# yefeng22222/RUB_MIMO

Measured on AMD Instinct MI355X. Metric: complex IQ samples/s through 4x4 MMSE detect; EVM-dB delta vs CPU ref, higher is better.
Workload: dtype fp32 (complex64; fp64 weight solve)

## Files before the change

rub_mimo_amd/csrc/engine.cpp:

```cpp
#include <mutex>

#include "engine_internal.hpp"

namespace {

thread_local std::string g_err;

std::mutex g_tw_mu;
float2 *g_tw = nullptr;
int g_tw_dev = -1;

}

namespace mimo {

int host_fail(int code, const char *msg) {
  g_err = msg;
  return code;
}

int get_twiddles(float2 **out) {
  std::lock_guard<std::mutex> lk(g_tw_mu);
  int dev = 0;
  HIPCHK(hipGetDevice(&dev));
// ... 163 lines not shown
  h->siso_tx = cfg->siso_tx; h->siso_rx = cfg->siso_rx;
  h->thr = cfg->plateau_threshold;
  h->cfo = cfg->cfo_correct != 0;
  h->qam = make_qam(q);
  h->acb = (uint64_t)h->SL * (h->nac * N + 4);
  h->txl = (uint64_t)h->pid * h->SL;
  h->win_len = h->acb + h->txl;
  h->dn = 1.0f / sqrtf((float)h->M_occ);
  h->ls_scale = h->dn / (float)h->nac;
  h->nv_norm = (h->nac >= 2) ? ((double)h->dn * (double)h->dn /
                                ((double)h->M_occ * N * N * (h->nac - 1)))
                             : 0.0;
  uint32_t F = 1;
  while (F < 2 * h->SL + h->M - 1 || F < 2 * h->M) F <<= 1;
  h->search_ls = F <= 16384 && search_ls_supported(ilog2(F), ilog2(h->M));
  if (!h->search_ls) {
    F = 1;
    while (F < h->SL + h->M - 1) F <<= 1;
    if (F > 8192) F = 8192;
    if (F < 2 * h->M) F = 2 * h->M;
  }
  h->F = F; h->log2F = ilog2(F);
  h->lagc = F - h->M + 1;
  h->n_lagc = (h->SL + h->lagc - 1) / h->lagc;
  h->n_slots = N * h->nac + 1;
  if (hip_stream) {
    h->stream = (hipStream_t)hip_stream;
  } else {
    if (hipStreamCreateWithFlags(&h->stream, hipStreamNonBlocking) != hipSuccess) {
      delete h;
      return fail(MIMO_ERR_HIP, "hipStreamCreate failed");
    }
    h->own_stream = true;
  }
  {
    int dev = 0, ncu = 0;
    if (hipGetDevice(&dev) == hipSuccess &&
        hipDeviceGetAttribute(&ncu, hipDeviceAttributeMultiprocessorCount, dev) == hipSuccess &&
        ncu > 0)
      h->n_cu = (uint32_t)ncu;
  }
  rc = get_twiddles(&h->tw);
  if (!rc) rc = build_codes(h->codes, h->M, N, h->nac, h->p.data(), cfg->s0_bits, cfg->s1_bits,
                            h->log2F, true, h->stream);
  if (rc) { mimo_rx_destroy(h); return rc; }
  uint32_t m_s0 = 0;
  for (uint32_t i = 0; i < h->M; i += 2) if (h->p[i] != MIMO_SC_NULL) m_s0++;
  std::vector<float> vs(h->n_slots);
  const double FF = (double)F * (double)F, MM = (double)h->M * (double)h->M;
  vs[0] = (float)((double)m_s0 / (MM * FF));
  for (uint32_t sl = 1; sl < h->n_slots; sl++) vs[sl] = (float)(1.0 / ((double)h->M * FF));
  if (ls_window_supported(h->log2M, h->nac, false)) {
    const uint32_t T = h->M / 8;
    std::vector<int8_t> sw(sign.size());
    for (size_t row = 0; row < (size_t)N * h->nac; row++)
      for (uint32_t lt = 0; lt < T; lt++)
        for (uint32_t e = 0; e < 8; e++) sw[row * h->M + 8 * lt + e] = sign[row * h->M + lt + T * e];
    if (h->s1sign_w.ensure(sw.size()) != hipSuccess ||
        hipMemcpy(h->s1sign_w.p, sw.data(), sw.size(), hipMemcpyHostToDevice) != hipSuccess) {
      mimo_rx_destroy(h);
      return fail(MIMO_ERR_HIP, "table upload failed");
    }
  }
  if (h->vscale.ensure(h->n_slots) != hipSuccess || h->s1sign.ensure(sign.size()) != hipSuccess ||
      h->occ.ensure(h->M) != hipSuccess ||
      hipMemcpy(h->vscale.p, vs.data(), sizeof(float) * vs.size(), hipMemcpyHostToDevice) !=
          hipSuccess ||
      hipMemcpy(h->s1sign.p, sign.data(), sign.size(), hipMemcpyHostToDevice) != hipSuccess ||
      hipMemcpy(h->occ.p, h->occ_index.data(), sizeof(int32_t) * h->M, hipMemcpyHostToDevice) !=
          hipSuccess) {
    mimo_rx_destroy(h);
    return fail(MIMO_ERR_HIP, "table upload failed");
  }
  *out = h;
  return MIMO_OK;
}

int mimo_rx_destroy(mimo_rx *h) {
  if (!h) return MIMO_OK;
  if (h->stream) (void)hipStreamSynchronize(h->stream);
  close_debug_files(h);
  for (auto &e : h->timer.ev) {
    (void)hipEventDestroy(e.second.first);
    (void)hipEventDestroy(e.second.second);
  }
  for (auto &g : h->graphs)
    if (g.exec) (void)hipGraphExecDestroy(g.exec);
  if (h->own_stream && h->stream) (void)hipStreamDestroy(h->stream);
  delete h;
  return MIMO_OK;
}

int mimo_rx_set_callback(mimo_rx *h, mimo_rx_symbol_cb cb, void *user) {
  if (!h) return fail(MIMO_ERR_ARG, "null handle");
  h->cb = cb;
  h->user = user;
  return MIMO_OK;
}

int mimo_rx_set_siso(mimo_rx *h, uint32_t tx, uint32_t rx) {
  if (!h || tx >= h->N || rx >= h->N) return fail(MIMO_ERR_ARG, "siso index out of range");
  if (tx != h->siso_tx || rx != h->siso_rx) invalidate_graph(h);
  h->siso_tx = tx;
  h->siso_rx = rx;
  return MIMO_OK;
}

int mimo_rx_set_grid_cus(mimo_rx *h, uint32_t n_cu) {
  if (!h) return fail(MIMO_ERR_ARG, "null handle");
  int dev = 0, ncu = 0;
  if (n_cu == 0 && hipGetDevice(&dev) == hipSuccess &&
// ... 263 lines not shown
```

rub_mimo_amd/csrc/engine_diag.cpp:

```cpp
#include "engine_internal.hpp"

namespace mimo {

const DiagEnv &diag_env() {
  static const DiagEnv env = [] {
    auto on = [](const char *name) { const char *e = getenv(name); return e && e[0] == '1'; };
    DiagEnv d{};
    const char *e = getenv("RMIMO_SC_DIAG");
    d.sc_diag = e ? atoi(e) : 0;
    d.sc_prof = on("RMIMO_SC_PROF");
    d.sc_one_phase = on("RMIMO_SC_PHASES");
    d.sc_count = on("RMIMO_SC_COUNT");
    d.sc_count_items = d.sc_count && getenv("RMIMO_SC_COUNT")[1] == '+';
    e = getenv("RMIMO_LS_FORM");
    d.ls_terms = e && strcmp(e, "terms") == 0;
    d.dec_prof = on("RMIMO_DEC_PROF");
    d.cfo_debug = on("RMIMO_CFO_DEBUG");
    d.no_graph = on("RMIMO_NO_GRAPH") || d.sc_prof || d.dec_prof;
    return d;
  }();
  return env;
}

int diag_sc_prof_arm(mimo_rx *h, bool screen, hipStream_t s, unsigned long long **prof) {
  if (!diag_env().sc_prof) return MIMO_OK;
  if (!h->sc_prof.p) HIPCHK(h->sc_prof.ensure(32));
  HIPCHK(hipMemsetAsync(h->sc_prof.p, 0, 32 * sizeof(unsigned long long), s));
  HIPCHK(hipMemsetAsync(h->sc_prof.p + 8, 0xFF, sizeof(unsigned long long), s));
  if (screen) HIPCHK(hipMemsetAsync(h->sc_prof.p, 0xFF, sizeof(unsigned long long), s));
  *prof = h->sc_prof.p;
  return MIMO_OK;
}

int diag_sc_count(mimo_rx *h, uint32_t F, uint64_t nchunks, bool screen, uint32_t hot_cap,
                  hipStream_t s) {
  if (!diag_env().sc_count) return MIMO_OK;
  hipStreamCaptureStatus cst = hipStreamCaptureStatusNone;
  (void)hipStreamIsCapturing(s, &cst);
  if (cst != hipStreamCaptureStatusNone) return MIMO_OK;
  uint32_t q[2] = {0, 0};
  HIPCHK(hipMemcpyAsync(q, h->ws.queue.p, sizeof(q), hipMemcpyDeviceToHost, s));
  HIPCHK(hipStreamSynchronize(s));
  fprintf(stderr, "sc_count hot_items %u (screen %d, frames %u, chunks %llu)\n", q[1],
          screen ? 1 : 0, F, (unsigned long long)nchunks);
  if (!diag_env().sc_count_items || !screen) return MIMO_OK;
  const uint32_t n = std::min(q[1], hot_cap);
  std::vector<ScHot> hv(n);
  std::vector<unsigned long long> mn((size_t)F * nchunks), mx((size_t)F * nchunks);
  HIPCHK(hipMemcpyAsync(hv.data(), h->ws.hot.p, sizeof(ScHot) * n, hipMemcpyDeviceToHost, s));
  HIPCHK(hipMemcpyAsync(mn.data(), h->ws.scr_min.p, sizeof(unsigned long long) * mn.size(),
                        hipMemcpyDeviceToHost, s));
  HIPCHK(hipMemcpyAsync(mx.data(), h->ws.scr_max.p, sizeof(unsigned long long) * mx.size(),
                        hipMemcpyDeviceToHost, s));
  HIPCHK(hipStreamSynchronize(s));
  for (uint32_t i = 0; i < n; i++) {
    const ScHot &it = hv[i];
    const size_t ci = (size_t)it.f * nchunks + it.chunk;
    const long long lo = (long long)mn[ci] - it.w0, hi = (long long)mx[ci] - it.w0;
    const long long a0 = std::max<long long>(0, (lo - (long long)h->cp - 2) / kScIterLen);
    const long long a1 = std::min<long long>(kScSpan / kScIterLen - 1, hi / kScIterLen);
    fprintf(stderr, "sc_item %u f %u chunk %llu w0 %lld c0 %lld unproven [%lld, %lld] (%lld) "
            "iterations %lld-%lld\n", i, it.f, (unsigned long long)it.chunk, (long long)it.w0,
            (long long)it.c0, lo, hi, hi - lo + 1, a0, a1);
  }
  return MIMO_OK;
}

int diag_sc_prof_report(mimo_rx *h, bool screen, hipStream_t s) {
  if (!diag_env().sc_prof) return MIMO_OK;
  if (screen) {
    unsigned long long v[32];
// ... 8 lines not shown
            v[6], v[6] ? (double)v[10] / v[6] / 100.0 : 0.0,
            v[12] ? (double)v[11] / v[12] / 100.0 : 0.0, v[12], (double)(v[13] >> 32) / 100.0,
            (v[13] >> 24) & 0xFF, (double)(v[13] & 0xFFFFFF) / 100.0, v[14] >> 32,
            v[14] & 0xFFFFFFFFull, v[15]);
    const double np = v[4] ? (double)v[4] : 1.0;
    fprintf(stderr, "exact_split record %.2f us setup %.2f us iterations %.2f us (%.2f per pass) "
            "start offset avg %.2f max %.2f us | per iteration: ring %.2f scan %.2f walk %.2f us "
            "(first iteration's ring %.2f us per pass; guarded fills %llu)\n",
            v[20] / np / 100.0, v[21] / np / 100.0,
            v[22] / np / 100.0, v[23] / np, (v[26] / np - (double)v[0]) / 100.0,
            (double)(v[25] - v[0]) / 100.0, v[23] ? v[16] / (double)v[23] / 100.0 : 0.0,
            v[23] ? v[17] / (double)v[23] / 100.0 : 0.0, v[23] ? v[18] / (double)v[23] / 100.0 : 0.0,
            v[19] / np / 100.0, v[24]);
    fprintf(stderr, "exact_windows max per iteration %llu, iterations with >= 2 windows %llu "
            "(their passes' max duration %.2f us)\n", v[27], v[28], (double)v[29] / 100.0);
  } else {
    unsigned long long v[20];
    HIPCHK(hipMemcpyAsync(v, h->sc_prof.p, sizeof(v), hipMemcpyDeviceToHost, s));
    HIPCHK(hipStreamSynchronize(s));
    const double it = v[0] ? (double)v[0] : 1.0;
    fprintf(stderr, "sc_prof items %llu skipped %llu antenna_passes %llu cycles/item rows %.0f "
            "words %.0f resolve %.0f total %.0f wall_us/item %.2f span_us %.2f max_item_us %.2f "
            "last_start_us %.2f\n", v[0], v[6], v[1],
            v[2] / it, v[3] / it, v[4] / it, v[5] / it, v[7] / it / 100.0,
            (double)(v[9] - v[8]) / 100.0, v[10] / 100.0, (double)(v[11] - v[8]) / 100.0);
    fprintf(stderr, "sc_prof phases/item warm %.0f A %.0f scan %.0f B %.0f run %.0f | resolve "
            "passes %llu chain cycles/pass %.0f samples/pass %.1f\n",
            v[12] / it, v[13] / it, v[14] / it, v[15] / it, v[16] / it, v[17],
            v[17] ? (double)v[18] / v[17] : 0.0, v[17] ? (double)v[19] / v[17] : 0.0);
  }
  return MIMO_OK;
}

int diag_dec_prof_arm(mimo_rx *h, hipStream_t s, unsigned long long **prof) {
  if (!diag_env().dec_prof) return MIMO_OK;
  if (!h->sc_prof.p) HIPCHK(h->sc_prof.ensure(28));
  HIPCHK(hipMemsetAsync(h->sc_prof.p, 0, 8 * sizeof(unsigned long long), s));
  *prof = h->sc_prof.p;
  return MIMO_OK;
}

int diag_dec_prof_report(mimo_rx *h, hipStream_t s) {
  if (!diag_env().dec_prof) return MIMO_OK;
  unsigned long long v[8];
  HIPCHK(hipMemcpyAsync(v, h->sc_prof.p, sizeof(v), hipMemcpyDeviceToHost, s));
  HIPCHK(hipStreamSynchronize(s));
  const double it = v[0] ? (double)v[0] : 1.0;
  fprintf(stderr, "dec_prof items %llu cycles/item load %.0f fft %.0f apply %.0f reduce %.0f "
          "| stream split: pass0 %.0f fetch %.0f subfft %.0f\n",
          v[0], v[1] / it, v[2] / it, v[3] / it, v[4] / it, v[5] / it, v[6] / it, v[7] / it);
  return MIMO_OK;
}

int diag_cfo_frames(mimo_rx *h, uint32_t F, hipStream_t s) {
  if (!diag_env().cfo_debug || !h->cfo) return MIMO_OK;
  std::vector<FrameInfo> fi(F);
  HIPCHK(hipMemcpyAsync(fi.data(), h->ws.info.p, sizeof(FrameInfo) * F, hipMemcpyDeviceToHost, s));
  HIPCHK(hipStreamSynchronize(s));
  for (uint32_t f = 0; f < F; f++)
    fprintf(stderr, "cfo_dbg f %u status %d base %lld i0 %u eps %.9f E %lld\n", f, (int)fi[f].status,
            (long long)fi[f].base, fi[f].i0, (double)fi[f].cfo_eps, (long long)fi[f].cfo_E);
  return MIMO_OK;
}

}
```

rub_mimo_amd/csrc/engine_internal.hpp:

```cpp
#pragma once

#include <hip/hip_runtime.h>

#include <algorithm>
#include <array>
#include <cmath>
#include <cstdio>
#include <cstdlib>
#include <cstring>
#include <string>
#include <utility>
#include <vector>

#include "../../include/mimo_rx.h"
#include "kernels.hpp"

using namespace mimo;

#pragma GCC visibility push(hidden)
namespace mimo {

inline int fail(int code, const std::string &msg) { return host_fail(code, msg.c_str()); }

#define HIPCHK(x)                                                                       \
// ... 83 lines not shown
    return b.ensure(cnt);
  }
  uint32_t rec_frames = 0;
  uint64_t rec_stride = 0;
  DevBuf<unsigned long long> trig, keys;
  DevBuf<ScRecord> rec;
  DevBuf<FrameInfo> info;
  DevBuf<float2> G, W;
  DevBuf<float> gain;
  DevBuf<double> nvp, evm_part, evm_out, evm_chunk, lspart;
  DevBuf<uint32_t> evm_cnt;
  DevBuf<uint32_t> nrec;
  DevBuf<float2> lsq;
  DevBuf<unsigned long long> n_exact;
  DevBuf<uint32_t> queue;
  DevBuf<ScHot> hot;
  DevBuf<uint32_t> scr_flag;
  DevBuf<unsigned long long> scr_min, scr_max;
  DevBuf<unsigned long long> cand;
  DevBuf<unsigned long long> certfail;
  DevBuf<float2> spec;
  DevBuf<float2> wide;
  DevBuf<float2> cfo_iq;
  DevBuf<double> cfo_eps;
};

}
#pragma GCC visibility pop

struct mimo_rx {
  uint32_t M = 0, cp = 0, SL = 0, N = 0, nac = 0, pid = 0;
  uint32_t M_null = 0, M_pilot = 0, M_data = 0, M_occ = 0;
  int log2M = 0, log2F = 0;
  uint32_t F = 0, lagc = 0, n_lagc = 0, n_slots = 0;
  bool search_ls = false;
  bool cfo = false;
  uint32_t n_cu = 256;
  int det = 0;
  float noise_var = -1.0f;
  int keep_bias = 1;
  uint32_t siso_tx = 0, siso_rx = 0;
  double thr = 0.95;
  Qam qam{};
  uint64_t acb = 0, txl = 0, win_len = 0;
  float dn = 1.0f, ls_scale = 1.0f;
  double nv_norm = 0.0;
  std::vector<uint8_t> p;
  std::vector<int32_t> occ_index;
  hipStream_t stream = nullptr;
  bool own_stream = false;
  float2 *tw = nullptr;
  Codes codes;
  DevBuf<float> vscale;
  DevBuf<int8_t> s1sign, s1sign_w;
  DevBuf<int32_t> occ;
  Workspace ws;
  uint32_t last_frames = 0, last_max_out = 0;
  int last_decode_path = MIMO_DECODE_NONE;
  int last_cfo_mode = 0;
  uint32_t last_layout = 0;
  DevBuf<float> nu;
  DevBuf<float2> sic_T, sic_C;
  DevBuf<uint8_t> sic_order, sic_ok;
  DevBuf<float> sic_nu;
  DevBuf<float2> capbuf;
  uint64_t cap_len = 0, total = 0, origin = 0;
  uint64_t trim_clo = ~0ull;
  DevBuf<uint32_t> probe;
  int state = MIMO_STATE_SEEK_PLATEAU;
  uint64_t nsp = 0;
  bool have_sync = false, have_est = false;
  FrameInfo sinfo{};
  DevBuf<float2> symbuf;
  std::vector<float2> symhost;
  mimo_rx_symbol_cb cb = nullptr;
  void *user = nullptr;
  std::string dbg_dir;
  std::vector<FILE *> dbg_fsc;
  DevBuf<float> dbg_y, dbg_corr;
  DevBuf<unsigned long long> sc_prof;
  StageTimer timer;
  struct GraphEntry {
    mimo_batch key{};
    hipStream_t stream = nullptr;
    uint64_t gen = 0;
    hipGraphExec_t exec = nullptr;
    uint64_t used = 0;
  };
  std::array<GraphEntry, 4> graphs{};
  uint64_t graph_tick = 0;
};

struct mimo_tx {
  uint32_t M = 0, cp = 0, SL = 0, N = 0, nac = 0, M_occ = 0;
  int log2M = 0;
  float dn = 1.0f;
  hipStream_t stream = nullptr;
  Codes codes;
  std::vector<float2> s0, s1;
  DevBuf<int32_t> occ_list;
  DevBuf<float2> din, dout;
  float2 *tw = nullptr;
};

#pragma GCC visibility push(hidden)
namespace mimo {

int get_twiddles(float2 **out);
Qam make_qam(uint32_t order);
int validate_sctype(const uint8_t *p, uint32_t M, uint32_t *n0, uint32_t *n1, uint32_t *n2);
int build_codes(Codes &c, uint32_t M, uint32_t N, uint32_t nac, const uint8_t *p,
                const uint8_t *s0_bits, const uint8_t *s1_bits, int log2F, bool spectra,
                hipStream_t s);
int copy_W(mimo_rx *h, uint32_t f, float *W);
int copy_corr(mimo_rx *h, uint32_t F, uint32_t *corr, uint32_t *s0);

int ensure_workspace(mimo_rx *h, uint32_t F, uint64_t chunks);
double sc_band(uint32_t M);
struct SyncRequest {
  uint64_t chunk_lo;
  bool reset_trig;
  uint32_t fpc;
  const uint64_t *ref_starts;
  uint32_t ref_stride;
  bool zero_keys;
};
int run_sync(mimo_rx *h, const Capture &c, uint32_t F, const SyncRequest &q, hipStream_t s);
int run_estimate(mimo_rx *h, const Capture &c, uint32_t F, bool keys_zeroed, CfoBatchArgs *cfo,
                 float *corr_trace, hipStream_t s);
struct DecodeRequest {
  uint32_t max_out;
  float2 *out_sym;
  uint8_t *out_idx;
  uint32_t layout;
  int ref_mode;
  const uint8_t *ref_idx;
  uint64_t ref_seed, frame_id0;
  uint32_t n_caps;
  const double *cfo_fold_part;
};
int run_decode(mimo_rx *h, const Capture &c, uint32_t F, const DecodeRequest &q, hipStream_t s);

void invalidate_graph(mimo_rx *h);

struct DiagEnv {
  int sc_diag;
  bool sc_prof;
  bool sc_one_phase;
  bool sc_count;
  bool sc_count_items;
  bool ls_terms;
  bool dec_prof;
  bool cfo_debug;
  bool no_graph;
};
const DiagEnv &diag_env();
int diag_sc_prof_arm(mimo_rx *h, bool screen, hipStream_t s, unsigned long long **prof);
int diag_sc_count(mimo_rx *h, uint32_t F, uint64_t nchunks, bool screen, uint32_t hot_cap,
                  hipStream_t s);
int diag_sc_prof_report(mimo_rx *h, bool screen, hipStream_t s);
int diag_dec_prof_arm(mimo_rx *h, hipStream_t s, unsigned long long **prof);
int diag_dec_prof_report(mimo_rx *h, hipStream_t s);
int diag_cfo_frames(mimo_rx *h, uint32_t F, hipStream_t s);

}
#pragma GCC visibility pop
```

rub_mimo_amd/csrc/engine_stages.cpp:

```cpp
#include "engine_internal.hpp"

namespace mimo {

int ensure_workspace(mimo_rx *h, uint32_t F, uint64_t chunks) {
  Workspace &w = h->ws;
  if (F > w.rec_frames) {
    HIPCHK(w.grow(w.trig, F));
    HIPCHK(w.grow(w.keys, (size_t)F * h->N * h->n_slots));
    HIPCHK(w.grow(w.info, F));
    HIPCHK(w.grow(w.G, (size_t)F * h->M * h->N * h->N));
    HIPCHK(w.grow(w.W, (size_t)F * h->M * h->N * h->N));
    HIPCHK(w.grow(w.gain, (size_t)F * h->M));
    HIPCHK(w.grow(w.nvp, (size_t)F * h->N * h->N * ((h->M + 255) / 256)));
    HIPCHK(w.grow(w.evm_out, (size_t)F * h->N * 3));
    HIPCHK(w.grow(w.evm_chunk, (size_t)F * kEvmChunks * h->N * 3));
    HIPCHK(w.grow(w.evm_cnt, F));
    HIPCHK(w.grow(w.nrec, F));
    HIPCHK(hipMemset(w.evm_cnt.p, 0, sizeof(uint32_t) * F));
    w.rec_frames = F;
    HIPCHK(w.grow(w.rec, (size_t)F * w.rec_stride));
  }
  if (chunks > w.rec_stride) {
    const uint64_t nc = std::max<uint64_t>(chunks, w.rec_stride * 2);
    ScRecord *np = nullptr;
// ... 101 lines not shown
        sa.chunk_lo = c1;
        sa.chunk_hi = nchunks;
        sa.trig = w.trig.p;
        launch_sc_screen(sa, F, s);
        ScArgs a2 = a;
        a2.item_lo = w.queue.p + 2;
        launch_sc_exact(a2, s);
        if (a.diag & 32) launch_sc_finalize(a2, s);
      }
    } else {
      launch_sc(a, F, h->n_cu, s);
      launch_sc_hot(a, s);
    }
    if ((rc = diag_sc_count(h, F, nchunks, screen, hot_cap, s))) return rc;
    h->timer.end(0, e, s);
    if ((rc = diag_sc_prof_report(h, screen, s))) return rc;
  }
  PlateauArgs pa{};
  set_capture(pa, c);
  pa.trig = w.trig.p; pa.rec = w.rec.p; pa.rec_stride = w.rec_stride; pa.chunk_len = K;
  pa.N = h->N; pa.M = h->M; pa.SL = h->SL; pa.thr = h->thr; pa.win_len = h->win_len;
  pa.band = sc_band(h->M);
  pa.info = w.info.p;
  pa.fpc = fpc; pa.nchunks = nchunks;
  pa.cand = stream ? w.cand.p : nullptr;
  pa.certfail = stream ? w.certfail.p : nullptr;
  pa.ref_starts = q.ref_starts;
  pa.ref_stride = q.ref_stride ? q.ref_stride : fpc;
  hipEvent_t e = h->timer.begin(s);
  if (stream) launch_stream_walk(pa, F, s);
  else launch_plateau(pa, F, s);
  h->timer.end(1, e, s);
  HIPCHK(hipGetLastError());
  return MIMO_OK;
}

int run_estimate(mimo_rx *h, const Capture &c, uint32_t F, bool keys_zeroed, CfoBatchArgs *cfo,
                 float *corr_trace, hipStream_t s) {
  Workspace &w = h->ws;
  if (!keys_zeroed)
    HIPCHK(hipMemsetAsync(w.keys.p, 0, sizeof(unsigned long long) * F * h->N * h->n_slots, s));
  SearchArgs sa{};
  set_capture(sa, c);
  sa.N = h->N; sa.M = h->M; sa.SL = h->SL; sa.n_slots = h->n_slots;
  sa.lagc = h->lagc; sa.n_lagc = h->n_lagc;
  sa.codespec = h->codes.codespec.p; sa.vscale = h->vscale.p;
  sa.codespec_w = h->codes.codespec_w.p;
  sa.info = w.info.p; sa.keys = w.keys.p; sa.tw = h->tw;
  sa.corr_trace = corr_trace;
  LsArgs la{};
  set_capture(la, c);
  la.N = h->N; la.M = h->M; la.nac = h->nac; la.n_slots = h->n_slots;
  la.keys = w.keys.p; la.s1sign = h->s1sign.p; la.occ_index = h->occ.p;
  la.s1sign_w = h->s1sign_w.p;
  la.keep_bias = h->keep_bias; la.scale = h->ls_scale; la.info = w.info.p;
  la.n_groups = (h->nac + kLsCodesPerGroup - 1) / kLsCodesPerGroup;
  la.n_nvp = h->N * h->N * ((h->M + 255) / 256);
  la.G = w.G.p; la.nv_part = w.nvp.p; la.tw = h->tw;
  auto cfo_stage2 = [&](int rot_window) {
    cfo->keys = w.keys.p; cfo->n_slots = h->n_slots; cfo->rot_window = rot_window;
    launch_cfo_batch(*cfo, F, 2, s);
  };
  if (h->search_ls) {
    const bool ls_win = !diag_env().ls_terms && ls_window_supported(h->log2M, h->nac, cfo != nullptr);
    if (!ls_win) {
      HIPCHK(w.grow(w.lsq, (size_t)F * h->N * h->N * h->nac * h->M));
      sa.s1sign = h->s1sign.p; sa.lsq = w.lsq.p; sa.nac = h->nac;
      la.lsq = w.lsq.p;
    }
    sa.xcd_order = 1;
    sa.cfo_part = (cfo && cfo->fold) ? cfo->part : nullptr;
    hipEvent_t e = h->timer.begin(s);
    launch_search_ls(sa, h->log2F, h->log2M, F, s);
    h->timer.end(2, e, s);
    if (cfo) {
      cfo_stage2(0);
      la.cfo_part = cfo->part;
      if (ls_win) la.cfo_fold = cfo->fold;
    }
    e = h->timer.begin(s);
    if (!ls_win) launch_ls_combine_q(la, F, s);
    else if (!launch_ls_window(la, h->log2M, F, s))
      return fail(MIMO_ERR_UNSUPPORTED, "ls_window_kernel: no instance for this geometry");
    h->timer.end(3, e, s);
  } else {
    hipEvent_t e = h->timer.begin(s);
    launch_search(sa, h->log2F, F, s);
    h->timer.end(2, e, s);
    if (cfo) cfo_stage2(1);
    HIPCHK(w.grow(w.lspart, (size_t)F * h->N * h->N * la.n_groups * 3 * h->M));
    la.part = w.lspart.p;
    e = h->timer.begin(s);
    launch_ls(la, h->log2M, F, s);
    h->timer.end(3, e, s);
  }
  WeightArgs wa{};
  wa.N = h->N; wa.M = h->M; wa.M_occ = h->M_occ; wa.nac = h->nac; wa.SL = h->SL;
  wa.n_slots = h->n_slots; wa.detector = h->det; wa.noise_var = h->noise_var;
  wa.nv_norm = h->nv_norm; wa.occ_index = h->occ.p; wa.G = w.G.p; wa.W = w.W.p;
  wa.gain = w.gain.p; wa.nv_part = w.nvp.p; wa.n_nvp = la.n_nvp; wa.keys = w.keys.p;
  wa.win_len = h->win_len;
  wa.info = w.info.p;
  hipEvent_t e = h->timer.begin(s);
  launch_weights(wa, F, s);
  h->timer.end(4, e, s);
  HIPCHK(hipGetLastError());
  return MIMO_OK;
}

int run_decode(mimo_rx *h, const Capture &c, uint32_t F, const DecodeRequest &q, hipStream_t s) {
  Workspace &w = h->ws;
  const uint32_t max_out = q.max_out;
  int rc = ensure_workspace(h, F, 0);
  if (rc || max_out == 0) return rc;
  DecodeArgs d{};
  set_capture(d, c);
  d.N = h->N; d.M = h->M; d.cp = h->cp; d.SL = h->SL; d.M_occ = h->M_occ;
  d.detector = h->det; d.siso_tx = h->siso_tx; d.siso_rx = h->siso_rx; d.dn = h->dn;
  d.occ_index = h->occ.p; d.W = w.W.p; d.gain = w.gain.p; d.G = w.G.p; d.info = w.info.p;
  d.max_out = max_out; d.out_sym = q.out_sym; d.out_idx = q.out_idx;
  if (q.layout == MIMO_LAYOUT_SYMBOL_MAJOR) {
    d.o_ts = h->M_occ;
    d.o_ss = (uint64_t)h->N * h->M_occ;
  } else {
    d.o_ts = (uint64_t)max_out * h->M_occ;
    d.o_ss = h->M_occ;
  }
  d.ref_mode = q.ref_mode; d.ref_idx = q.ref_idx; d.ref_seed = q.ref_seed;
  d.frame_id0 = q.frame_id0;
  d.qam = h->qam; d.tw = h->tw;
  d.n_frames = F; d.n_cu = h->n_cu;
  d.n_caps = q.n_caps ? q.n_caps : F; d.n_refs = F;
  d.all_occ = (h->M_occ == h->M) ? 1 : 0;
  if ((rc = diag_dec_prof_arm(h, s, &d.prof))) return rc;
  hipEvent_t e = h->timer.begin(s);
  d.nrec = w.nrec.p;
  d.cpe = h->cfo ? (q.cfo_fold_part ? 2 : 1) : 0;
// ... 38 lines not shown
```

rub_mimo_amd/csrc/est_kernels.hip:

```cpp
#include <cstdlib>
#include <cstring>

#include "est_common.hpp"
#include "fft.hpp"
#include "fft_reg.hpp"
#include "kernels.hpp"

namespace mimo {

MIMO_DEV void corr_trace_put(const SearchArgs &a, uint32_t f, uint32_t r, uint32_t slot,
                             int64_t lag, float v) {
  if (a.corr_trace && lag >= 0 && lag < (int64_t)a.SL)
    a.corr_trace[(((uint64_t)f * a.N + r) * a.n_slots + slot) * a.SL + lag] = v;
}

template <int LOG2F>
__global__ __launch_bounds__(kEstT) void search_kernel(SearchArgs a) {
  constexpr int F = 1 << LOG2F;
  extern __shared__ __attribute__((aligned(16))) float2 lds[];
  __shared__ unsigned long long s_key;
  const uint32_t f = blockIdx.y;
  const FrameInfo &I = a.info[f];
  if (I.status != 0) return;
  const int tid = threadIdx.x;
// ... 616 lines not shown
    if (valid) {
      const uint32_t ac = s0 + u - 1, code = ac / a.N, tx = ac % a.N;
      const auto sg = sgpr_ptr(a.s1sign + ((size_t)tx * a.nac + code) * M);
      const auto q = sgpr_ptr(reinterpret_cast<v2f *>(a.lsq) +
                              ((((uint64_t)f * a.N + r) * a.N + tx) * a.nac + code) * M);
#pragma unroll
      for (int e = 0; e < 8; e++) {
        const uint32_t k = (uint32_t)reg_index<LOG2M, 8>((int)lt, e);
        const int8_t sv = sg[k];
        const float sgn = (float)sv;
        const v2f term = sv ? xw[e] * v2f{sgn, sgn} : v2f{0.0f, 0.0f};
        ls_term_store(&q[k], term);
      }
    }
  } else {
    float2 *twm = reinterpret_cast<float2 *>(lds_raw) + lds_padded_len(F);
    fill_twiddles_lds<LOG2M, T>(twm, a.tw);
    float2 win[NL];
#pragma unroll
    for (int e = 0; e < NL; e++) {
      const int i = tid + e * T, uu = i / M, j = i % M;
      const int64_t n = (uu ? w1v : w0) + j;
      const bool ok = (uu ? valid1 : valid0) && n >= 0 && n < L;
      win[e] = ok ? xs.at(n) : make_float2(0.0f, 0.0f);
      if constexpr (CFO) {
        const v2f ph = phasor_cycles(cfo_lds.nu * (double)(n - I.base));
        const v2f w = vmul(v2f{win[e].x, win[e].y}, ph);
        win[e] = make_float2(w.x, w.y);
      }
    }
    float2 *lb = reinterpret_cast<float2 *>(buf);
#pragma unroll
    for (int e = 0; e < NL; e++) {
      const int i = tid + e * T, uu = i / M, j = i % M;
      lb[uu * PBM + lds_pad(j)] = win[e];
    }
    __syncthreads();
    fft_lds_twl<LOG2M, T, 2, false>(lb, twm, tid);
#pragma unroll
    for (int e = 0; e < NL; e++) {
      const int i = tid + e * T, uu = i / M, k = i % M;
      if (!(uu ? valid1 : valid0)) continue;
      const uint32_t ac = s0 + uu - 1, code = ac / a.N, tx = ac % a.N;
      const int8_t *sg = a.s1sign + ((size_t)tx * a.nac + code) * M;
      float2 *q = a.lsq + ((((uint64_t)f * a.N + r) * a.N + tx) * a.nac + code) * M;
      const float2 Xk = lb[uu * PBM + lds_pad(k)];
      const int sgn = sg[k];
      const float2 t = sgn > 0 ? Xk : (sgn < 0 ? cneg(Xk) : make_float2(0.0f, 0.0f));
      q[k] = t;
    }
  }
}

template <int LOG2M, bool SC16, bool CFO>
__global__ __launch_bounds__((1 << LOG2M) / 8) __attribute__((amdgpu_waves_per_eu(4)))
void ls_window_kernel(LsArgs a) {
  using PM = RegPlan<LOG2M, 8>;
  constexpr int M = 1 << LOG2M, T = PM::T, NW = T / 64;
  static_assert(T % 64 == 0, "whole waves");
  extern __shared__ __attribute__((aligned(16))) float2 lds_raw[];
  v2f *buf = reinterpret_cast<v2f *>(lds_raw);
  constexpr bool S2REG = LOG2M <= 11;
  double *s2l = reinterpret_cast<double *>(lds_raw + reg_image_len<LOG2M, 8>()) + threadIdx.x;
  v2f *pa = buf, *pb = buf + reg_image_len<LOG2M, 8>();
  __shared__ double red[M / 64];
  const uint32_t rt = blockIdx.x, f = blockIdx.y;
  const FrameInfo &I = a.info[f];
  if (I.status != 0) return;
  const uint32_t N = a.N, r = rt / N, t = rt % N, nac = a.nac;
  const int lt = threadIdx.x, lane = lt & 63;
  const uint32_t wv = __builtin_amdgcn_readfirstlane((uint32_t)lt >> 6);
  const int64_t L = (int64_t)a.frame_len;
  const auto xs = iq_row<SC16>(a.iq, a.iq_scale, ((uint64_t)I.cap * N + r) * a.stride);
  const unsigned long long *kp = a.keys + ((uint64_t)f * N + r) * a.n_slots + 1 + t;
  __shared__ v2f s_rot[CFO ? kLsRotCodes : 1];
  __shared__ double s_nu1, s_nu2;
  __shared__ v2f s_step;
  v2f q_lt = v2f{1.0f, 0.0f};
  if constexpr (CFO) {
    if (lt == 0) {
      const double nu2 = cfo_stage_eps(a.cfo_part, f, 2) / (double)M;
      s_nu2 = nu2;
      if (rt == 0) {
        const double eps = cfo_stage_eps(a.cfo_part, f, 1) + nu2 * M;
        const_cast<FrameInfo &>(I).cfo_eps = (float)eps;
        const_cast<FrameInfo &>(I).cfo_E = cfo_fixed_freq(eps, M);
      }
      s_nu1 = a.cfo_fold ? cfo_stage_eps(a.cfo_part, f, 1) / (double)M : 0.0;
      s_step = phasor_cycles(s_nu1 * (double)(M / 8));
    }
    __syncthreads();
    const double nu1 = s_nu1, nu2 = s_nu2;
    for (uint32_t c = lt; c < nac; c += T) {
      const double k = (double)key_index(kp[(uint64_t)c * N]);
      s_rot[c] = phasor_cycles(nu1 * k + nu2 * (k + 0.5 * (double)M));
    }
    q_lt = phasor_cycles(nu1 * (double)lt);
    __syncthreads();
  }
  auto load_win = [&](uint32_t c, v2f *xw) {
    const int64_t wb = I.base + (int64_t)key_index(kp[(uint64_t)c * N]);
    if (wb >= 0 && wb + M <= L) {
      const auto xr = xs.row((uint64_t)wb);
#pragma unroll
      for (int e = 0; e < 8; e++) {
        const float2 v = xr.at(reg_index<LOG2M, 8>(lt, e));
        xw[e] = v2f{v.x, v.y};
      }
    } else {
#pragma unroll
      for (int e = 0; e < 8; e++) {
        const int64_t n = wb + reg_index<LOG2M, 8>(lt, e);
        const float2 v = xs.at(n < 0 ? 0 : (n >= L ? L - 1 : n));
        xw[e] = (n >= 0 && n < L) ? v2f{v.x, v.y} : v2f{0.0f, 0.0f};
      }
    }
  };
  auto derotate = [&](uint32_t c, v2f *xw) {
    v2f rb = vmul(s_rot[c], q_lt);
    const v2f st = s_step;
#pragma unroll
    for (int e = 0; e < 8; e++) {
      xw[e] = vmul(xw[e], rb);
      rb = vmul(rb, st);
    }
  };
  auto load_sign = [&](uint32_t c) {
    return *reinterpret_cast<const uint2 *>(a.s1sign_w + ((size_t)t * nac + c) * M + 8 * lt);
  };
  v2f wm[PM::NTW > 0 ? PM::NTW : 1];
  reg_twiddles<LOG2M, 8>(wm, a.tw, lt);
  double sr[8], si[8], s2r[S2REG ? 8 : 1];
#pragma unroll
  for (int e = 0; e < 8; e++) {
    sr[e] = si[e] = 0.0;
    if constexpr (S2REG) s2r[e] = 0.0;
    else s2l[e * T] = 0.0;
  }
  v2f xn[8];
  load_win(0, xn);
  uint2 sn = load_sign(0);
  for (uint32_t c = 0; c < nac; c++) {
    v2f xw[8];
#pragma unroll
    for (int e = 0; e < 8; e++) xw[e] = xn[e];
    const uint2 sv = sn;
    if (c + 1 < nac) {
      load_win(c + 1, xn);
      sn = load_sign(c + 1);
    }
    if constexpr (CFO) derotate(c, xw);
    reg_compute<LOG2M, 8, 0, false>(xw, wm);
    if constexpr (S2REG) {
      reg_rest_pp<LOG2M, 8, 1, false>(pa, pb, xw, wm, lt);
      if constexpr ((PM::NP - 1) & 1) {
        v2f *tmp = pa;
        pa = pb;
        pb = tmp;
      }
    } else {
      reg_rest_lay<LOG2M, 8, 1, false, true>(buf, xw, wm, lt);
    }
#pragma unroll
    for (int e = 0; e < 8; e++) {
      const int8_t s8 = (int8_t)(((e < 4 ? sv.x : sv.y) >> (8 * (e & 3))) & 0xFFu);
      const float sgn = (float)s8;
      const v2f term = s8 ? xw[e] * v2f{sgn, sgn} : v2f{0.0f, 0.0f};
      sr[e] += (double)term.x;
      si[e] += (double)term.y;
      if constexpr (S2REG) s2r[e] += (double)term.x * term.x + (double)term.y * term.y;
      else s2l[e * T] += (double)term.x * term.x + (double)term.y * term.y;
    }
  }
  const double bias = (a.keep_bias && r == t) ? 1.0 : 0.0;
#pragma unroll
  for (int e = 0; e < 8; e++) {
    const uint32_t k = (uint32_t)reg_index<LOG2M, 8>(lt, e);
    const bool occ = a.occ_index[k] >= 0;
    a.G[(((uint64_t)f * M + k) * N + r) * N + t] =
        occ ? make_float2((float)((bias + sr[e]) * a.scale), (float)(si[e] * a.scale))
            : make_float2(0.0f, 0.0f);
    const double s2 = S2REG ? s2r[S2REG ? e : 0] : s2l[e * T];
    double nv = occ ? s2 - (sr[e] * sr[e] + si[e] * si[e]) / (double)nac : 0.0;
#pragma unroll
    for (int off = 32; off > 0; off >>= 1) nv += __shfl_xor(nv, off);
    if (lane == 0) red[(64 * wv + T * e) / 64] = nv;
  }
  __syncthreads();
  for (int b = lt; b < M / 256; b += T)
    a.nv_part[(uint64_t)f * a.n_nvp + (uint64_t)rt * (M / 256) + b] =
        red[4 * b] + red[4 * b + 1] + red[4 * b + 2] + red[4 * b + 3];
  (void)NW;
}

template <int LOG2F>
static void search_dispatch(const SearchArgs &a, int log2F, uint32_t nf, hipStream_t s) {
  if constexpr (LOG2F <= 13) {
    if (log2F == LOG2F) {
      const size_t shm = sizeof(float2) * lds_padded_len(1 << LOG2F);
      dim3 grid(a.n_slots * a.N * a.n_lagc, nf);
      if constexpr (LOG2F >= 10) {
        (void)hipFuncSetAttribute((const void *)search_reg_kernel<LOG2F>,
                                  hipFuncAttributeMaxDynamicSharedMemorySize, (int)shm);
        hipLaunchKernelGGL(search_reg_kernel<LOG2F>, grid, dim3((1 << LOG2F) / 16), shm, s, a);
      } else {
        (void)hipFuncSetAttribute((const void *)search_kernel<LOG2F>,
                                  hipFuncAttributeMaxDynamicSharedMemorySize, (int)shm);
        hipLaunchKernelGGL(search_kernel<LOG2F>, grid, dim3(kEstT), shm, s, a);
      }
      return;
    }
    search_dispatch<LOG2F + 1>(a, log2F, nf, s);
  }
}

void launch_search(const SearchArgs &a, int log2F, uint32_t n_frames, hipStream_t s) {
  search_dispatch<7>(a, log2F, n_frames, s);
}

template <int LOG2F, int D>
static bool search_ls_try(const SearchArgs &a, int log2F, int log2M, uint32_t nf, hipStream_t s) {
  if constexpr (LOG2F <= 14) {
    if constexpr (D <= 3) {
      constexpr int LOG2M = LOG2F - D;
      if (log2F == LOG2F && log2M == LOG2M) {
        if (nf) {
          const size_t shm = sizeof(float2) * (lds_padded_len(1 << LOG2F) + (1 << LOG2M) / 2);
          void (*kern)(SearchArgs) = nullptr;
          if constexpr (LOG2F >= 10) {
            if (search_ls_wave_enabled() && a.codespec_w)
              kern = a.cfo_part ? (a.sc16 ? search_ls_wave_kernel<LOG2F, LOG2M, true, true>
                                          : search_ls_wave_kernel<LOG2F, LOG2M, false, true>)
                                : (a.sc16 ? search_ls_wave_kernel<LOG2F, LOG2M, true>
                                          : search_ls_wave_kernel<LOG2F, LOG2M, false>);
          }
          if (!kern)
            kern = a.cfo_part ? (a.sc16 ? search_ls_kernel<LOG2F, LOG2M, true, true>
                                        : search_ls_kernel<LOG2F, LOG2M, false, true>)
                              : (a.sc16 ? search_ls_kernel<LOG2F, LOG2M, true>
                                        : search_ls_kernel<LOG2F, LOG2M, false>);
          (void)hipFuncSetAttribute((const void *)kern,
                                    hipFuncAttributeMaxDynamicSharedMemorySize, (int)shm);
          dim3 grid(((a.n_slots + 1) / 2) * a.N, nf);
          hipLaunchKernelGGL(kern, grid, dim3((1 << LOG2F) / 16), shm, s, a);
        }
        return true;
      }
      return search_ls_try<LOG2F, D + 1>(a, log2F, log2M, nf, s);
    } else {
      return search_ls_try<LOG2F + 1, 1>(a, log2F, log2M, nf, s);
    }
  }
  return false;
}

bool search_ls_wave_enabled() {
  static const bool block = [] { const char *e = getenv("RMIMO_SEARCH_FORM"); return e && strcmp(e, "block") == 0; }();
  return !block;
}

bool search_ls_supported(int log2F, int log2M) {
  return search_ls_try<10, 1>(SearchArgs{}, log2F, log2M, 0, nullptr);
}

bool launch_search_ls(const SearchArgs &a, int log2F, int log2M, uint32_t n_frames, hipStream_t s) {
  return search_ls_try<10, 1>(a, log2F, log2M, n_frames, s);
}

bool ls_window_supported(int log2M, uint32_t nac, bool cfo) {
  return log2M >= 9 && log2M <= 12 && (!cfo || nac <= (uint32_t)kLsRotCodes);
}

bool launch_ls_window(const LsArgs &a, int log2M, uint32_t n_frames, hipStream_t s) {
  if (!ls_window_supported(log2M, a.nac, a.cfo_part != nullptr) || !a.s1sign_w) return false;
  if (!n_frames) return true;
  void (*kern)(LsArgs) = nullptr;
  size_t shm = 0;
  int T = 0;
  const bool cfo = a.cfo_part != nullptr;
  switch (log2M) {
#define LSW(L2)                                                                             \
  case L2:                                                                                  \
    kern = cfo ? (a.sc16 ? ls_window_kernel<L2, true, true> : ls_window_kernel<L2, false, true>) \
               : (a.sc16 ? ls_window_kernel<L2, true, false> : ls_window_kernel<L2, false, false>); \
    shm = sizeof(float2) * reg_image_len<L2, 8>() *                                          \
              (L2 > 11 ? 1 : 2) + (L2 > 11 ? sizeof(double) * (1 << L2) : 0);              \
    T = (1 << L2) / 8;                                                                      \
    break;
    LSW(9) LSW(10) LSW(11) LSW(12)
#undef LSW
  }
  (void)hipFuncSetAttribute((const void *)kern, hipFuncAttributeMaxDynamicSharedMemorySize, (int)shm);
  hipLaunchKernelGGL(kern, dim3(a.N * a.N, n_frames), dim3(T), shm, s, a);
  return true;
}

}
```

rub_mimo_amd/csrc/kernels.hpp:

```cpp
#pragma once

#include <hip/hip_runtime.h>
#include <stdint.h>

#include "common.hpp"

namespace mimo {

struct ScRecord {
  unsigned long long n_cand;
  unsigned long long start[kMaxStreams];
  long long pos0;
  uint32_t found;
  uint32_t pad;
};
constexpr int kScSpan = 16384;
constexpr int kScThreads = 256;
constexpr int kScIterLen = 4096;
constexpr int kScAmbMax = 256;
inline uint64_t sc_chunk_len(uint32_t cp) { return kScSpan - ((uint64_t)cp + 2 + 15) / 16 * 16; }
size_t sc_lds_bytes(uint32_t M, uint32_t N);
size_t sc_table_bytes(uint32_t M);

struct ScHot {
// ... 78 lines not shown
  const float2 *iq;
  int sc16;
  float iq_scale;
  uint64_t stride, frame_len;
  uint32_t N, M, SL;
  double thr, band;
  uint64_t win_len;
  FrameInfo *info;
  uint32_t fpc;
  uint64_t nchunks;
  const unsigned long long *cand;
  unsigned long long *certfail;
  const uint64_t *ref_starts;
  uint32_t ref_stride;
};
void launch_plateau(const PlateauArgs &a, uint32_t n_frames, hipStream_t s);
void launch_stream_walk(const PlateauArgs &a, uint32_t n_caps, hipStream_t s);
void launch_sc_trace(const float2 *iq, uint64_t stride, uint32_t rows, uint32_t M, int64_t lo,
                     int64_t hi, float *out, hipStream_t s);

struct SearchArgs {
  const float2 *iq;
  int sc16;
  float iq_scale;
  uint64_t stride, frame_len;
  uint32_t N, M, SL, n_slots;
  uint32_t lagc, n_lagc;
  const float2 *codespec;
  const float2 *codespec_w;
  const float *vscale;
  const FrameInfo *info;
  unsigned long long *keys;
  const float2 *tw;
  const int8_t *s1sign;
  float2 *lsq;
  uint32_t nac;
  uint32_t xcd_order;
  const double *cfo_part;
  float *corr_trace;
};
void launch_search(const SearchArgs &a, int log2F, uint32_t n_frames, hipStream_t s);
bool launch_search_ls(const SearchArgs &a, int log2F, int log2M, uint32_t n_frames, hipStream_t s);
bool search_ls_supported(int log2F, int log2M);
bool search_ls_wave_enabled();

struct LsArgs {
  const float2 *iq;
  uint64_t stride, frame_len;
  int sc16;
  float iq_scale;
  uint32_t N, M, nac, n_slots;
  const unsigned long long *keys;
  const int8_t *s1sign;
  const int8_t *s1sign_w;
  const int32_t *occ_index;
  int keep_bias;
  float scale;
  const FrameInfo *info;
  float2 *G;
  double *part;
  uint32_t n_groups;
  double *nv_part;
  uint32_t n_nvp;
  const float2 *tw;
  const float2 *lsq;
  const double *cfo_part;
  uint32_t M_cfo;
  int cfo_fold;
};
constexpr uint32_t kLsCodesPerGroup = 4;
void launch_ls(const LsArgs &a, int log2M, uint32_t n_frames, hipStream_t s);
void launch_ls_combine_q(const LsArgs &a, uint32_t n_frames, hipStream_t s);
bool launch_ls_window(const LsArgs &a, int log2M, uint32_t n_frames, hipStream_t s);
bool ls_window_supported(int log2M, uint32_t nac, bool cfo);

struct WeightArgs {
  uint32_t N, M, M_occ, nac, SL, n_slots;
  int detector;
  float noise_var;
  double nv_norm;
  const int32_t *occ_index;
  const float2 *G;
  float2 *W;
  float *gain;
  const double *nv_part;
  uint32_t n_nvp;
  const unsigned long long *keys;
  uint64_t win_len;
  FrameInfo *info;
};
void launch_weights(const WeightArgs &a, uint32_t n_frames, hipStream_t s);

struct CfoBatchArgs {
  const float2 *iq;
  float2 *out;
  uint64_t stride, frame_len, len;
  uint64_t win;
  uint32_t N, M, cp, SL;
  uint32_t n_codes;
  uint32_t n_data;
  uint32_t n_slots;
  int rot_window;
  int fold;
  FrameInfo *info;
  const unsigned long long *keys;
  double *part;
};
size_t cfo_batch_part_doubles(uint32_t n_frames);
void launch_cfo_batch(const CfoBatchArgs &a, uint32_t n_frames, int stage, hipStream_t s);
void launch_cfo_batch_rot2(const CfoBatchArgs &a, uint32_t n_frames, hipStream_t s);

struct DecodeArgs {
  const float2 *iq;
  int sc16;
  float iq_scale;
  uint64_t stride, frame_len;
  uint32_t N, M, cp, SL, M_occ;
  int detector;
  uint32_t siso_tx, siso_rx;
  float dn;
  const int32_t *occ_index;
  const float2 *W;
// ... 180 lines not shown
```

Measured before the change: 261.5 billion.

## Streamline LS window kernel: cached keys, sign-bit XOR, occupancy bitmask, batched reductions

Caches per-code key indices in shared memory so the next window's key is read from LDS instead of global memory. Stores the S1 signs as 0x80/0 sign-bit masks and applies them with a byte permute plus XOR rather than an int-to-float convert and multiply. Replaces the per-subcarrier occ_index lookups with a precomputed per-thread occupancy bitmask, and batches the eight noise-variance wavefront reductions so the shuffles interleave. Zeroing of out-of-range samples is deferred until after the load, and optional clock-based profiling instrumentation is added behind a compile flag. The extra LDS array and the new device table add setup cost, and dropping sign value 0 (now treated as +1) assumes every sign entry is ±1.

```diff
diff --git a/rub_mimo_amd/csrc/engine.cpp b/rub_mimo_amd/csrc/engine.cpp
--- a/rub_mimo_amd/csrc/engine.cpp
+++ b/rub_mimo_amd/csrc/engine.cpp
@@ -239,11 +239,16 @@
   for (uint32_t sl = 1; sl < h->n_slots; sl++) vs[sl] = (float)(1.0 / ((double)h->M * FF));
   if (ls_window_supported(h->log2M, h->nac, false)) {
     const uint32_t T = h->M / 8;
-    std::vector<int8_t> sw(sign.size());
+    std::vector<uint8_t> sw(sign.size()), ow(T, 0);
     for (size_t row = 0; row < (size_t)N * h->nac; row++)
       for (uint32_t lt = 0; lt < T; lt++)
-        for (uint32_t e = 0; e < 8; e++) sw[row * h->M + 8 * lt + e] = sign[row * h->M + lt + T * e];
-    if (h->s1sign_w.ensure(sw.size()) != hipSuccess ||
+        for (uint32_t e = 0; e < 8; e++)
+          sw[row * h->M + 8 * lt + e] = sign[row * h->M + lt + T * e] < 0 ? 0x80 : 0;
+    for (uint32_t lt = 0; lt < T; lt++)
+      for (uint32_t e = 0; e < 8; e++)
+        if (h->occ_index[lt + T * e] >= 0) ow[lt] |= (uint8_t)(1u << e);
+    if (h->s1sign_w.ensure(sw.size()) != hipSuccess || h->occ_w.ensure(ow.size()) != hipSuccess ||
+        hipMemcpy(h->occ_w.p, ow.data(), ow.size(), hipMemcpyHostToDevice) != hipSuccess ||
         hipMemcpy(h->s1sign_w.p, sw.data(), sw.size(), hipMemcpyHostToDevice) != hipSuccess) {
       mimo_rx_destroy(h);
       return fail(MIMO_ERR_HIP, "table upload failed");
diff --git a/rub_mimo_amd/csrc/engine_diag.cpp b/rub_mimo_amd/csrc/engine_diag.cpp
--- a/rub_mimo_amd/csrc/engine_diag.cpp
+++ b/rub_mimo_amd/csrc/engine_diag.cpp
@@ -16,7 +16,10 @@
     d.ls_terms = e && strcmp(e, "terms") == 0;
     d.dec_prof = on("RMIMO_DEC_PROF");
     d.cfo_debug = on("RMIMO_CFO_DEBUG");
-    d.no_graph = on("RMIMO_NO_GRAPH") || d.sc_prof || d.dec_prof;
+#ifdef MIMO_LS_PROFILE
+    d.ls_prof = on("RMIMO_LS_PROF");
+#endif
+    d.no_graph = on("RMIMO_NO_GRAPH") || d.sc_prof || d.dec_prof || d.ls_prof;
     return d;
   }();
   return env;
@@ -131,6 +134,40 @@
   return MIMO_OK;
 }
 
+int diag_ls_prof_arm(mimo_rx *h, uint32_t F, hipStream_t s, unsigned long long **prof) {
+  if (!diag_env().ls_prof) return MIMO_OK;
+  const size_t n = kLsProfHead + (size_t)F * h->N * h->N;
+  HIPCHK(h->ls_prof.ensure(n));
+  HIPCHK(hipMemsetAsync(h->ls_prof.p, 0, n * sizeof(unsigned long long), s));
+  HIPCHK(hipMemsetAsync(h->ls_prof.p + kLsProfHead - 1, 0xFF, sizeof(unsigned long long), s));
+  *prof = h->ls_prof.p;
+  return MIMO_OK;
+}
+
+int diag_ls_prof_report(mimo_rx *h, uint32_t F, hipStream_t s) {
+  if (!diag_env().ls_prof || !h->ls_prof.p) return MIMO_OK;
+  std::vector<unsigned long long> v(kLsProfHead + (size_t)F * h->N * h->N);
+  HIPCHK(hipMemcpyAsync(v.data(), h->ls_prof.p, sizeof(unsigned long long) * v.size(),
+                        hipMemcpyDeviceToHost, s));
+  HIPCHK(hipStreamSynchronize(s));
+  if (!v[0]) return MIMO_OK;
+  const double wg = (double)v[0], pc = wg * (double)h->nac;
+  fprintf(stderr, "ls_prof workgroups %llu codes %u cycles/workgroup total %.0f prologue %.0f "
+          "epilogue %.0f | cycles/code window_wait %.0f prefetch_issue %.0f pass0 %.0f "
+          "exchanges %.0f (store %.0f barrier %.0f load %.0f; exchange 1 %.0f 2 %.0f 3 %.0f) "
+          "later_passes %.0f sign_accumulate %.0f\n", v[0], h->nac, v[11] / wg, v[10] / wg,
+          v[9] / wg, v[1] / pc, v[2] / pc, v[3] / pc, (v[4] + v[5] + v[6]) / pc, v[4] / pc,
+          v[5] / pc, v[6] / pc, v[12] / pc, v[13] / pc, v[14] / pc, v[7] / pc, v[8] / pc);
+  std::vector<unsigned long long> end;
+  for (size_t i = kLsProfHead; i < v.size(); i++)
+    if (v[i]) end.push_back(v[i] - v[kLsProfHead - 1]);
+  if (end.empty()) return MIMO_OK;
+  std::sort(end.begin(), end.end());
+  fprintf(stderr, "ls_prof workgroup end times min %.2f median %.2f max %.2f us\n",
+          end.front() / 100.0, end[end.size() / 2] / 100.0, end.back() / 100.0);
+  return MIMO_OK;
+}
+
 int diag_cfo_frames(mimo_rx *h, uint32_t F, hipStream_t s) {
   if (!diag_env().cfo_debug || !h->cfo) return MIMO_OK;
   std::vector<FrameInfo> fi(F);
diff --git a/rub_mimo_amd/csrc/engine_internal.hpp b/rub_mimo_amd/csrc/engine_internal.hpp
--- a/rub_mimo_amd/csrc/engine_internal.hpp
+++ b/rub_mimo_amd/csrc/engine_internal.hpp
@@ -159,7 +159,8 @@
   float2 *tw = nullptr;
   Codes codes;
   DevBuf<float> vscale;
-  DevBuf<int8_t> s1sign, s1sign_w;
+  DevBuf<int8_t> s1sign;
+  DevBuf<uint8_t> s1sign_w, occ_w;
   DevBuf<int32_t> occ;
   Workspace ws;
   uint32_t last_frames = 0, last_max_out = 0;
@@ -186,6 +187,7 @@
   std::vector<FILE *> dbg_fsc;
   DevBuf<float> dbg_y, dbg_corr;
   DevBuf<unsigned long long> sc_prof;
+  DevBuf<unsigned long long> ls_prof;
   StageTimer timer;
   struct GraphEntry {
     mimo_batch key{};
@@ -258,6 +260,7 @@
   bool sc_count_items;
   bool ls_terms;
   bool dec_prof;
+  bool ls_prof;
   bool cfo_debug;
   bool no_graph;
 };
@@ -268,6 +271,8 @@
 int diag_sc_prof_report(mimo_rx *h, bool screen, hipStream_t s);
 int diag_dec_prof_arm(mimo_rx *h, hipStream_t s, unsigned long long **prof);
 int diag_dec_prof_report(mimo_rx *h, hipStream_t s);
+int diag_ls_prof_arm(mimo_rx *h, uint32_t F, hipStream_t s, unsigned long long **prof);
+int diag_ls_prof_report(mimo_rx *h, uint32_t F, hipStream_t s);
 int diag_cfo_frames(mimo_rx *h, uint32_t F, hipStream_t s);
 
 }
diff --git a/rub_mimo_amd/csrc/engine_stages.cpp b/rub_mimo_amd/csrc/engine_stages.cpp
--- a/rub_mimo_amd/csrc/engine_stages.cpp
+++ b/rub_mimo_amd/csrc/engine_stages.cpp
@@ -177,7 +177,7 @@
   set_capture(la, c);
   la.N = h->N; la.M = h->M; la.nac = h->nac; la.n_slots = h->n_slots;
   la.keys = w.keys.p; la.s1sign = h->s1sign.p; la.occ_index = h->occ.p;
-  la.s1sign_w = h->s1sign_w.p;
+  la.s1sign_w = h->s1sign_w.p; la.occ_w = h->occ_w.p;
   la.keep_bias = h->keep_bias; la.scale = h->ls_scale; la.info = w.info.p;
   la.n_groups = (h->nac + kLsCodesPerGroup - 1) / kLsCodesPerGroup;
   la.n_nvp = h->N * h->N * ((h->M + 255) / 256);
@@ -203,11 +203,14 @@
       la.cfo_part = cfo->part;
       if (ls_win) la.cfo_fold = cfo->fold;
     }
+    int rc = MIMO_OK;
+    if (ls_win && (rc = diag_ls_prof_arm(h, F, s, &la.prof))) return rc;
     e = h->timer.begin(s);
     if (!ls_win) launch_ls_combine_q(la, F, s);
     else if (!launch_ls_window(la, h->log2M, F, s))
       return fail(MIMO_ERR_UNSUPPORTED, "ls_window_kernel: no instance for this geometry");
     h->timer.end(3, e, s);
+    if (ls_win && (rc = diag_ls_prof_report(h, F, s))) return rc;
   } else {
     hipEvent_t e = h->timer.begin(s);
     launch_search(sa, h->log2F, F, s);
diff --git a/rub_mimo_amd/csrc/est_kernels.hip b/rub_mimo_amd/csrc/est_kernels.hip
--- a/rub_mimo_amd/csrc/est_kernels.hip
+++ b/rub_mimo_amd/csrc/est_kernels.hip
@@ -692,6 +692,45 @@
   }
 }
 
+#ifdef MIMO_LS_PROFILE
+#define LS_PROF(...) __VA_ARGS__
+#define LS_TICK(i)                              \
+  {                                             \
+    __builtin_amdgcn_sched_barrier(0);          \
+    const uint32_t n_ = (uint32_t)clock64();    \
+    pf[i] += n_ - pt;                           \
+    pt = n_;                                    \
+    __builtin_amdgcn_sched_barrier(0);          \
+  }
+template <int LOG2N, int PTS, int P, bool INV>
+MIMO_DEV void reg_rest_pp_prof(v2f *img0, v2f *img1, v2f *v, const v2f *w1, int tid,
+                               uint32_t *pf, uint32_t &pt) {
+  using PL = RegPlan<LOG2N, PTS>;
+  if constexpr (P < PL::NP) {
+    int t = tid;
+    asm volatile("" : "+v"(t));
+    constexpr int LAY = reg_ex_layout<LOG2N, PTS>(P - 1);
+    v2f *buf = ((P - 1) & 1) ? img1 : img0;
+    const uint32_t x0 = pt;
+    reg_store_lay<LOG2N, PTS, P - 1, LAY>(buf, v, t);
+    asm volatile("s_waitcnt lgkmcnt(0)" ::: "memory");
+    LS_TICK(4)
+    asm volatile("s_barrier" ::: "memory");
+    LS_TICK(5)
+    reg_load_lay<LOG2N, PTS, P, LAY>(buf, v, t);
+    asm volatile("s_waitcnt lgkmcnt(0)" ::: "memory");
+    LS_TICK(6)
+    pf[12 + (P - 1 < 2 ? P - 1 : 2)] += pt - x0;
+    reg_compute<LOG2N, PTS, P, INV>(v, w1);
+    LS_TICK(7)
+    reg_rest_pp_prof<LOG2N, PTS, P + 1, INV>(img0, img1, v, w1, tid, pf, pt);
+  }
+}
+#else
+#define LS_PROF(...)
+#define LS_TICK(i)
+#endif
+
 template <int LOG2M, bool SC16, bool CFO>
 __global__ __launch_bounds__((1 << LOG2M) / 8) __attribute__((amdgpu_waves_per_eu(4)))
 void ls_window_kernel(LsArgs a) {
@@ -707,6 +746,8 @@
   const uint32_t rt = blockIdx.x, f = blockIdx.y;
   const FrameInfo &I = a.info[f];
   if (I.status != 0) return;
+  LS_PROF(uint32_t pf[15] = {}; const unsigned long long pw0 = wall_clock64();
+          const uint32_t pt0 = (uint32_t)clock64(); uint32_t pt = pt0;)
   const uint32_t N = a.N, r = rt / N, t = rt % N, nac = a.nac;
   const int lt = threadIdx.x, lane = lt & 63;
   const uint32_t wv = __builtin_amdgcn_readfirstlane((uint32_t)lt >> 6);
@@ -717,6 +758,10 @@
   __shared__ double s_nu1, s_nu2;
   __shared__ v2f s_step;
   v2f q_lt = v2f{1.0f, 0.0f};
+  __shared__ uint32_t s_key[kLsRotCodes];
+  for (uint32_t c = lt; c < nac && c < (uint32_t)kLsRotCodes; c += T)
+    s_key[c] = key_index(kp[(uint64_t)c * N]);
+  if constexpr (!CFO) __syncthreads();
   if constexpr (CFO) {
     if (lt == 0) {
       const double nu2 = cfo_stage_eps(a.cfo_part, f, 2) / (double)M;
@@ -732,14 +777,18 @@
     __syncthreads();
     const double nu1 = s_nu1, nu2 = s_nu2;
     for (uint32_t c = lt; c < nac; c += T) {
-      const double k = (double)key_index(kp[(uint64_t)c * N]);
+      const double k = (double)s_key[c];
       s_rot[c] = phasor_cycles(nu1 * k + nu2 * (k + 0.5 * (double)M));
     }
     q_lt = phasor_cycles(nu1 * (double)lt);
     __syncthreads();
   }
-  auto load_win = [&](uint32_t c, v2f *xw) {
-    const int64_t wb = I.base + (int64_t)key_index(kp[(uint64_t)c * N]);
+  auto key_of = [&](uint32_t c) {
+    return c < (uint32_t)kLsRotCodes ? s_key[c] : key_index(kp[(uint64_t)c * N]);
+  };
+  const int64_t base = I.base;
+  auto load_win = [&](uint32_t key, v2f *xw) {
+    const int64_t wb = base + (int64_t)__builtin_amdgcn_readfirstlane(key);
     if (wb >= 0 && wb + M <= L) {
       const auto xr = xs.row((uint64_t)wb);
 #pragma unroll
@@ -752,8 +801,17 @@
       for (int e = 0; e < 8; e++) {
         const int64_t n = wb + reg_index<LOG2M, 8>(lt, e);
         const float2 v = xs.at(n < 0 ? 0 : (n >= L ? L - 1 : n));
-        xw[e] = (n >= 0 && n < L) ? v2f{v.x, v.y} : v2f{0.0f, 0.0f};
-      }
+        xw[e] = v2f{v.x, v.y};
+      }
+    }
+    return wb;
+  };
+  auto zero_outside = [&](int64_t wb, v2f *xw) {
+    if (wb >= 0 && wb + M <= L) return;
+#pragma unroll
+    for (int e = 0; e < 8; e++) {
+      const int64_t n = wb + reg_index<LOG2M, 8>(lt, e);
+      if (n < 0 || n >= L) xw[e] = v2f{0.0f, 0.0f};
     }
   };
   auto derotate = [&](uint32_t c, v2f *xw) {
@@ -778,21 +836,33 @@
     else s2l[e * T] = 0.0;
   }
   v2f xn[8];
-  load_win(0, xn);
+  int64_t wbn = load_win(key_of(0), xn);
   uint2 sn = load_sign(0);
-  for (uint32_t c = 0; c < nac; c++) {
+  uint32_t kn = nac > 1 ? key_of(1) : 0u;
+  LS_TICK(10)
+  auto one_code = [&](uint32_t c, bool more) __attribute__((always_inline)) {
+    LS_PROF(asm volatile("s_waitcnt vmcnt(0)" ::: "memory");)
+    LS_TICK(1)
     v2f xw[8];
 #pragma unroll
     for (int e = 0; e < 8; e++) xw[e] = xn[e];
+    zero_outside(wbn, xw);
     const uint2 sv = sn;
-    if (c + 1 < nac) {
-      load_win(c + 1, xn);
+    if (more) {
+      wbn = load_win(kn, xn);
       sn = load_sign(c + 1);
-    }
+      if (c + 2 < nac) kn = key_of(c + 2);
+    }
+    LS_TICK(2)
     if constexpr (CFO) derotate(c, xw);
     reg_compute<LOG2M, 8, 0, false>(xw, wm);
+    LS_TICK(3)
     if constexpr (S2REG) {
+#ifdef MIMO_LS_PROFILE
+      reg_rest_pp_prof<LOG2M, 8, 1, false>(pa, pb, xw, wm, lt, pf, pt);
+#else
       reg_rest_pp<LOG2M, 8, 1, false>(pa, pb, xw, wm, lt);
+#endif
       if constexpr ((PM::NP - 1) & 1) {
         v2f *tmp = pa;
         pa = pb;
@@ -803,34 +873,57 @@
     }
 #pragma unroll
     for (int e = 0; e < 8; e++) {
-      const int8_t s8 = (int8_t)(((e < 4 ? sv.x : sv.y) >> (8 * (e & 3))) & 0xFFu);
-      const float sgn = (float)s8;
-      const v2f term = s8 ? xw[e] * v2f{sgn, sgn} : v2f{0.0f, 0.0f};
+      const uint32_t sm = __builtin_amdgcn_perm(0u, e < 4 ? sv.x : sv.y,
+                                                0x000c0c0cu | ((uint32_t)(e & 3) << 24));
+      const v2f term = v2f{__uint_as_float(__float_as_uint(xw[e].x) ^ sm),
+                           __uint_as_float(__float_as_uint(xw[e].y) ^ sm)};
       sr[e] += (double)term.x;
       si[e] += (double)term.y;
       if constexpr (S2REG) s2r[e] += (double)term.x * term.x + (double)term.y * term.y;
       else s2l[e * T] += (double)term.x * term.x + (double)term.y * term.y;
     }
-  }
+    LS_TICK(8)
+  };
+  for (uint32_t c = 0; c + 1 < nac; c++) one_code(c, true);
+  one_code(nac - 1, false);
   const double bias = (a.keep_bias && r == t) ? 1.0 : 0.0;
+  const uint32_t occ_bits = a.occ_w[lt];
+  double nv[8];
 #pragma unroll
   for (int e = 0; e < 8; e++) {
     const uint32_t k = (uint32_t)reg_index<LOG2M, 8>(lt, e);
-    const bool occ = a.occ_index[k] >= 0;
+    const bool occ = (occ_bits >> e) & 1u;
     a.G[(((uint64_t)f * M + k) * N + r) * N + t] =
         occ ? make_float2((float)((bias + sr[e]) * a.scale), (float)(si[e] * a.scale))
             : make_float2(0.0f, 0.0f);
     const double s2 = S2REG ? s2r[S2REG ? e : 0] : s2l[e * T];
-    double nv = occ ? s2 - (sr[e] * sr[e] + si[e] * si[e]) / (double)nac : 0.0;
-#pragma unroll
-    for (int off = 32; off > 0; off >>= 1) nv += __shfl_xor(nv, off);
-    if (lane == 0) red[(64 * wv + T * e) / 64] = nv;
-  }
+    nv[e] = occ ? s2 - (sr[e] * sr[e] + si[e] * si[e]) / (double)nac : 0.0;
+  }
+#pragma unroll
+  for (int off = 32; off > 0; off >>= 1) {
+    double o[8];
+#pragma unroll
+    for (int e = 0; e < 8; e++) o[e] = __shfl_xor(nv[e], off);
+#pragma unroll
+    for (int e = 0; e < 8; e++) nv[e] += o[e];
+  }
+#pragma unroll
+  for (int e = 0; e < 8; e++)
+    if (lane == 0) red[(64 * wv + T * e) / 64] = nv[e];
   __syncthreads();
   for (int b = lt; b < M / 256; b += T)
     a.nv_part[(uint64_t)f * a.n_nvp + (uint64_t)rt * (M / 256) + b] =
         red[4 * b] + red[4 * b + 1] + red[4 * b + 2] + red[4 * b + 3];
   (void)NW;
+  LS_PROF(asm volatile("s_waitcnt vmcnt(0)" ::: "memory");)
+  LS_TICK(9)
+  LS_PROF(if (a.prof && lt == 0) {
+    atomicAdd(&a.prof[0], 1ull);
+    for (int i = 1; i < 15; i++)
+      atomicAdd(&a.prof[i], (unsigned long long)(i == 11 ? pt - pt0 : pf[i]));
+    atomicMin(&a.prof[kLsProfHead - 1], pw0);
+    a.prof[kLsProfHead + (uint64_t)f * gridDim.x + rt] = wall_clock64();
+  })
 }
 
 template <int LOG2F>
@@ -912,7 +1005,8 @@
 }
 
 bool launch_ls_window(const LsArgs &a, int log2M, uint32_t n_frames, hipStream_t s) {
-  if (!ls_window_supported(log2M, a.nac, a.cfo_part != nullptr) || !a.s1sign_w) return false;
+  if (!ls_window_supported(log2M, a.nac, a.cfo_part != nullptr) || !a.s1sign_w || !a.occ_w)
+    return false;
   if (!n_frames) return true;
   void (*kern)(LsArgs) = nullptr;
   size_t shm = 0;
diff --git a/rub_mimo_amd/csrc/kernels.hpp b/rub_mimo_amd/csrc/kernels.hpp
--- a/rub_mimo_amd/csrc/kernels.hpp
+++ b/rub_mimo_amd/csrc/kernels.hpp
@@ -154,7 +154,8 @@
   uint32_t N, M, nac, n_slots;
   const unsigned long long *keys;
   const int8_t *s1sign;
-  const int8_t *s1sign_w;
+  const uint8_t *s1sign_w;
+  const uint8_t *occ_w;
   const int32_t *occ_index;
   int keep_bias;
   float scale;
@@ -169,7 +170,9 @@
   const double *cfo_part;
   uint32_t M_cfo;
   int cfo_fold;
-};
+  unsigned long long *prof;
+};
+constexpr uint32_t kLsProfHead = 16;
 constexpr uint32_t kLsCodesPerGroup = 4;
 void launch_ls(const LsArgs &a, int log2M, uint32_t n_frames, hipStream_t s);
 void launch_ls_combine_q(const LsArgs &a, uint32_t n_frames, hipStream_t s);
```

Result: no change. 259.4 billion, median of 2 (-0.8%).
